# Algomorph/LevelSetFusion-Python

Measured on AMD Instinct MI355X. Metric: voxel-warp-updates/sec, higher is better.
Workload: dtype f32

## Files before the change

### include/lsf_hip.h

```cpp
#ifndef LSF_HIP_H
#define LSF_HIP_H

#include <stdint.h>

#ifdef __cplusplus
extern "C" {
#endif

#define LSF_ABI_VERSION 4
#define LSF_MAX_KERNEL_TAPS 31

#define LSF_ERR_BAD_ARGUMENT (-1)
#define LSF_ERR_BAD_DIMS (-2)
#define LSF_ERR_KERNEL_TOO_LONG (-3)
#define LSF_ERR_RCCL_UNAVAILABLE (-4)
#define LSF_ERR_RCCL_FAILED (-5)
#define LSF_ERR_NOT_RESIDENT (-6)

typedef struct lsf_grid {
    int32_t dims;
    int32_t nz, ny, nx;
    int32_t z_begin, z_end;
    int32_t z_global_offset;
    int32_t y_global_offset;
// ... 110 lines not shown
    double isomorphic_enforcement_factor_f64;
    float rate;
    float data_term_weight;
    float smoothing_term_weight;
    float level_set_term_weight;
    float isomorphic_enforcement_factor;
    float killing_c1;
    int32_t smoothing_method;
    int32_t data_method;
    int32_t level_set_enabled;
    int32_t energy_mode;
    int32_t zero_gradient_on_snap;
    int32_t reserved;
} lsf_slavcheva_params;

int lsf_slavcheva_gradient(const float *live, const float *canonical, const float *warp_prev_planar,
                           float *g_out_planar, const lsf_grid *grid, const lsf_slavcheva_params *params,
                           const lsf_gate *gate, lsf_iteration_record *record, const int32_t *band_list,
                           int64_t band_count, void *stream);

#define LSF_BAND_ALL 0
#define LSF_BAND_INTERIOR 1
#define LSF_BAND_BOUNDARY 2

int64_t lsf_band_scratch_elements(const lsf_grid *grid);
int lsf_band_count(const float *live, const float *canonical, const lsf_grid *grid, int32_t subset,
                   int32_t *scratch, int64_t *count_out, void *stream);
int lsf_band_list_fill(const float *live, const float *canonical, const lsf_grid *grid, int32_t subset,
                       const int32_t *scratch, int32_t *list, void *stream);

int64_t lsf_state_prepare_scratch_elements(const lsf_grid *grid);
int lsf_state_pack_needed(const float *live, float *state_a, float *state_b, const lsf_grid *grid, int32_t *scratch,
                          int32_t reach, int32_t invert, void *stream);

int lsf_band_list_fill_prepared(const lsf_grid *grid, int32_t subset, const int32_t *scratch, int32_t *list,
                                void *stream);
int lsf_state_prepare(const float *live, const float *canonical, float *state_a, float *state_b,
                      const lsf_grid *grid, int32_t *scratch, int64_t *counts_out, void *stream);
int lsf_state_pack(const float *live, const float *warp_planar, float *state_a, float *state_b,
                   const lsf_grid *grid, void *stream);
int lsf_state_unpack(const float *state, float *live_out, float *warp_planar_out, float *warp_interleaved_out,
                     const lsf_grid *grid, void *stream);
int64_t lsf_state_finalize_scratch_elements(const lsf_grid *grid);
int lsf_state_finalize(const float *state, const float *canonical, float *live_out, float *warp_planar_out,
                       float *warp_interleaved_out, const lsf_grid *grid, float lower_threshold,
                       double *statistics16, double *scratch, void *stream);
int lsf_planar_finalize(const float *live, const float *warp_planar, const float *canonical, float *live_out,
                        float *warp_interleaved_out, const lsf_grid *grid, float lower_threshold,
                        double *statistics16, double *scratch, void *stream);

int lsf_state_finalize_listed(const float *state, const float *canonical, float *live_out, float *warp_interleaved_out,
                              const lsf_grid *grid, const int32_t *const *band_lists, const int64_t *band_counts,
                              int32_t n_lists, int64_t opposite_count, int64_t first_opposite, float lower_threshold,
                              double *statistics16, double *scratch, const int32_t *skip_flag,
                              const lsf_iteration_record *guard_records, int32_t guard_count, float guard_limit,
                              void *stream);
int lsf_slavcheva_state_iteration(const float *state_in, const float *canonical, float *state_out,
                                  const lsf_grid *grid, const lsf_slavcheva_params *params, const lsf_gate *gate,
                                  lsf_iteration_record *record, const int32_t *band_list, int64_t band_count,
                                  int32_t band_subset, void *stream);

typedef struct lsf_band_box {
    int32_t origin;
    int32_t reserved;
    uint64_t mask;
} lsf_band_box;
// ... 292 lines not shown
```

### levelsetfusion-python_amd/_lib.py

```python
import ctypes
import os

import torch

from ._build import LIB_PATH

c_float_p = ctypes.c_void_p

MAX_KERNEL_TAPS = 31
ABI_VERSION = 4
HEADER_ABI_HASH = "bc02ed0838831b36"

ERRORS = {-1: "LSF_ERR_BAD_ARGUMENT", -2: "LSF_ERR_BAD_DIMS", -3: "LSF_ERR_KERNEL_TOO_LONG",
          -4: "LSF_ERR_RCCL_UNAVAILABLE", -5: "LSF_ERR_RCCL_FAILED", -6: "LSF_ERR_NOT_RESIDENT"}

SMOOTHING_TIKHONOV, SMOOTHING_KILLING = 0, 1
DATA_BASIC, DATA_THRESHOLDED_FDM = 0, 2
ENERGY_NONE, ENERGY_DIRECT, ENERGY_VECTORIZED = 0, 1, 2
GATE_HIERARCHICAL, GATE_SLAVCHEVA, GATE_OPEN = 0, 1, 2


class Grid(ctypes.Structure):
    _fields_ = [("dims", ctypes.c_int32), ("nz", ctypes.c_int32), ("ny", ctypes.c_int32), ("nx", ctypes.c_int32),
                ("z_begin", ctypes.c_int32), ("z_end", ctypes.c_int32), ("z_global_offset", ctypes.c_int32),
                ("y_global_offset", ctypes.c_int32), ("energy_z_begin", ctypes.c_int32), ("energy_z_end", ctypes.c_int32),
                ("ny_global", ctypes.c_int32), ("energy_y_begin", ctypes.c_int32), ("energy_y_end", ctypes.c_int32)]


BAND_ALL, BAND_INTERIOR, BAND_BOUNDARY = 0, 1, 2
RECORD_SLOTS = 8


class RecordSlot(ctypes.Structure):
    _fields_ = [("max_packed", ctypes.c_uint64), ("data_energy", ctypes.c_double),
                ("smoothing_energy", ctypes.c_double), ("level_set_energy", ctypes.c_double),
                ("pad", ctypes.c_uint64 * 508)]


class IterationRecord(ctypes.Structure):
    _fields_ = [("slot", RecordSlot * RECORD_SLOTS)]


RECORD_BYTES = ctypes.sizeof(IterationRecord)
SLOT_WORDS = ctypes.sizeof(RecordSlot) // 8
# ... 146 lines not shown
    "lsf_target_arch": (ctypes.c_char_p, []),
    "lsf_build_id": (ctypes.c_char_p, []),
    "lsf_abi_hash": (ctypes.c_char_p, []),
    "lsf_deinterleave": (ctypes.c_int, [_vp, _vp, _i64, _i32, _vp]),
    "lsf_interleave": (ctypes.c_int, [_vp, _vp, _i64, _i32, _vp]),
    "lsf_halo_copy": (ctypes.c_int, [_vp, _vp, _vp, _vp, _P(Grid), _i32, _i32, _i32, _i32, _i32, _vp]),
    "lsf_warp_field": (ctypes.c_int, [_vp, _vp, _vp, _P(Grid), _f32, _vp]),
    "lsf_warp_field_advanced": (ctypes.c_int, [_vp, _vp, _vp, _vp, _vp, _P(Grid), _i32, _vp]),
    "lsf_pack_live_gradient": (ctypes.c_int, [_vp, _vp, _P(Grid), _vp]),
    "lsf_restrict_mean": (ctypes.c_int, [_vp, _vp, _P(Grid), _i32, _vp]),
    "lsf_prolong_repeat": (ctypes.c_int, [_vp, _vp, _P(Grid), _vp]),
    "lsf_upsample2x_linear": (ctypes.c_int, [_vp, _vp, _P(Grid), _i32, _vp]),
    "lsf_downsample2x_linear": (ctypes.c_int, [_vp, _vp, _P(Grid), _i32, _vp]),
    "lsf_convolve_axis": (ctypes.c_int, [_vp, _vp, _vp, _P(Grid), _i32, _i32, _P(ctypes.c_double), _i32,
                                         _P(Gate), _vp]),
    "lsf_convolve_xy": (ctypes.c_int, [_vp, _vp, _P(Grid), _i32, _P(ctypes.c_double), _i32, _P(Gate), _vp]),
    "lsf_convolve_axis_update": (ctypes.c_int, [_vp, _vp, _vp, ctypes.c_float, _P(Grid), _i32, _i32, _P(ctypes.c_double),
                                                _i32, _P(Gate), _vp]),
    "lsf_convolve_xyz": (ctypes.c_int, [_vp, _vp, _vp, _f32, _P(Grid), _i32, _P(ctypes.c_double), _i32, _P(Gate),
                                        _vp]),
    "lsf_hier_iteration": (ctypes.c_int, [_vp, _vp, _vp, _vp, _vp, _P(Grid), _P(HierParams), _P(Gate), _vp, _vp]),
    "lsf_hier_update": (ctypes.c_int, [_vp, _vp, _P(Grid), _f32, _P(Gate), _vp, _vp]),
    "lsf_hier_level_run_2d": (ctypes.c_int, [_vp, _vp, _vp, _vp, _vp, _vp, _P(Grid), _P(HierParams), _P(ctypes.c_double),
                                            _i32, _vp, _i32, _i32, ctypes.c_float, _vp]),
    "lsf_slavcheva_gradient": (ctypes.c_int, [_vp, _vp, _vp, _vp, _P(Grid), _P(SlavchevaParams), _P(Gate), _vp,
                                              _vp, _i64, _vp]),
    "lsf_convolve_axis_listed": (ctypes.c_int, [_vp, _vp, _vp, _P(Grid), _i32, _i32, _P(ctypes.c_double), _i32,
                                                _P(Gate), _vp, _i64, _vp]),
    "lsf_state_prepare_scratch_elements": (ctypes.c_int64, [_P(Grid)]),
    "lsf_band_list_fill_prepared": (ctypes.c_int, [_P(Grid), _i32, _vp, _vp, _vp]),
    "lsf_state_prepare": (ctypes.c_int, [_vp, _vp, _vp, _vp, _P(Grid), _vp, _vp, _vp]),
    "lsf_state_pack": (ctypes.c_int, [_vp, _vp, _vp, _vp, _P(Grid), _vp]),
    "lsf_state_pack_needed": (ctypes.c_int, [_vp, _vp, _vp, _P(Grid), _vp, _i32, _i32, _vp]),
    "lsf_state_unpack": (ctypes.c_int, [_vp, _vp, _vp, _vp, _P(Grid), _vp]),
    "lsf_state_finalize_scratch_elements": (ctypes.c_int64, [_P(Grid)]),
    "lsf_state_finalize": (ctypes.c_int, [_vp, _vp, _vp, _vp, _vp, _P(Grid), _f32, _vp, _vp, _vp]),
    "lsf_planar_finalize": (ctypes.c_int, [_vp, _vp, _vp, _vp, _vp, _P(Grid), _f32, _vp, _vp, _vp]),
    "lsf_state_finalize_listed": (ctypes.c_int, [_vp, _vp, _vp, _vp, _P(Grid), _P(ctypes.c_void_p), _P(_i64), _i32,
                                                 _i64, _i64, _f32, _vp, _vp, _vp, _vp, _i32, _f32, _vp]),
    "lsf_slavcheva_state_iteration": (ctypes.c_int, [_vp, _vp, _vp, _P(Grid), _P(SlavchevaParams), _P(Gate), _vp,
                                                     _vp, _i64, _i32, _vp]),
    "lsf_band_boxes_scratch_elements": (ctypes.c_int64, [_P(Grid)]),
    "lsf_band_boxes_count": (ctypes.c_int, [_P(Grid), ctypes.c_int32, _vp, _vp, _vp, _vp]),
    "lsf_band_boxes_fill": (ctypes.c_int, [_P(Grid), ctypes.c_int32, _vp, _vp, _vp, _vp]),
    "lsf_band_boxes_canonical": (ctypes.c_int, [_vp, _P(Grid), _vp, ctypes.c_int64, _vp, _vp]),
    "lsf_slavcheva_state_iteration_boxes": (ctypes.c_int, [_vp, _vp, _vp, _P(Grid), _P(SlavchevaParams), _P(Gate), _vp, _vp,
                                                           _i64, _vp]),
    "lsf_state_run_begin": (ctypes.c_int, [_P(StateRun), _vp]),
    "lsf_state_run_finish": (ctypes.c_int, [_P(StateRun), _P(SlavchevaParams), _vp, _vp, _vp, _vp, _vp, _i32, _P(RunLoop), _vp,
                                            _f32, _vp, _vp, _vp, _vp, _P(StateRunResult), _vp]),
    "lsf_sobolev_run_finish": (ctypes.c_int, [_P(StateRun), _P(SlavchevaParams), _P(ctypes.c_double), _i32, _vp, _vp, _vp, _vp,
                                              _vp, _vp, _vp, _i32, _P(RunLoop), _vp, _f32, _vp, _vp, _vp, _vp,
                                              _P(StateRunResult), _vp]),
    "lsf_slab_run_begin": (ctypes.c_int, [_P(SlabRun), _vp]),
    "lsf_slab_run_finish": (ctypes.c_int, [_P(SlabRun), _vp, _P(SlavchevaParams), _vp, _vp, _vp, _vp, _vp, _i32, _vp, _vp, _vp,
                                           _P(StateRunResult), _vp]),
    "lsf_band_scratch_elements": (ctypes.c_int64, [_P(Grid)]),
    "lsf_band_count": (ctypes.c_int, [_vp, _vp, _P(Grid), _i32, _vp, _vp, _vp]),
    "lsf_band_list_fill": (ctypes.c_int, [_vp, _vp, _P(Grid), _i32, _vp, _vp, _vp]),
    "lsf_records_decode": (ctypes.c_int, [_vp, _i32, _i32, _i32, _vp, _vp, _vp, _vp]),
    "lsf_merge_sorted_runs": (ctypes.c_int, [_P(_vp), _P(_i64), _P(_vp), _P(_i64), _P(_vp), _i32, _vp]),
    "lsf_slab_unique_id": (ctypes.c_int, [ctypes.c_char_p, _vp]),
    "lsf_slab_comm_create": (ctypes.c_int, [ctypes.c_char_p, _vp, _i32, _i32, _P(_vp)]),
    "lsf_slab_comm_destroy": (ctypes.c_int, [_vp]),
    "lsf_slab_comm_info": (ctypes.c_int, [_vp, _P(_i32), _P(_i32)]),
    "lsf_slab_face_counts_begin": (ctypes.c_int, [_vp, _P(_i64)]),
# ... 76 lines not shown
```

### levelsetfusion-python_amd/csrc/lsf_device.h

```cpp
#pragma once

#include <hip/hip_runtime.h>
#include <cstdlib>
#include <stdint.h>

#include "../../include/lsf_hip.h"

namespace lsf {

constexpr int kWave = 64;
constexpr int kBlock = 256;
constexpr int kCuBlock = 1024;
constexpr int kMaxBlockWaves = kCuBlock / kWave;

struct FastDiv {
    unsigned d, m, l;
};

__host__ inline FastDiv make_fast_div(unsigned d) {
    FastDiv f;
    f.d = d;
    f.l = 0;
    while ((1ull << f.l) < d) ++f.l;
    f.m = (unsigned)(((1ull << 32) * ((1ull << f.l) - d)) / d + 1ull);
// ... 502 lines not shown
    return (float)__builtin_fma(-2.0, (double)a0, (double)ap + (double)am);
}

__device__ inline bool gate_closed(const lsf_gate& gate) {
    if (!gate.prev_record || gate.mode == LSF_GATE_OPEN) return false;
    unsigned long long p = 0ull;
#pragma unroll
    for (int k = 0; k < LSF_RECORD_SLOTS; ++k) {
        const unsigned long long q = gate.prev_record->slot[k].max_packed;
        p = q > p ? q : p;
    }
    if (p == 0ull) return true;
    float m = unpack_max_value(p);
    if (gate.mode == LSF_GATE_HIERARCHICAL) return m < gate.a;
    return !(gate.a < m && m < gate.b);
}

__device__ inline lsf_record_slot* record_slot(lsf_iteration_record* r) {
    return &r->slot[blockIdx.x % LSF_RECORD_SLOTS];
}

__device__ inline unsigned long long* record_max(lsf_iteration_record* r) {
    return reinterpret_cast<unsigned long long*>(&record_slot(r)->max_packed);
}

__host__ inline lsf_gate gate_or_open(const lsf_gate* gate) {
    return gate ? *gate : lsf_gate{nullptr, 0, 0.0f, 0.0f};
}

inline hipStream_t as_stream(void* s) { return reinterpret_cast<hipStream_t>(s); }

inline int launch_status() { return (int)hipGetLastError(); }

}
```

### levelsetfusion-python_amd/csrc/lsf_slavcheva.hip

```cpp
#include "lsf_device.h"

using namespace lsf;

#include "lsf_slavcheva_terms.h"

using namespace lsf::slav;

namespace {


template <int D, int SMOOTH, bool LEVELSET, int DATA, int ENERGY>
__device__ inline void voxel_gradient(const float* __restrict__ live, const float* __restrict__ canonical,
                                      const float* __restrict__ warp_prev, const Grid& g, const Params& p, int x,
                                      int y, int z, int i, float (&gv)[3], double (&en)[3]) {
    gv[0] = gv[1] = gv[2] = 0.0f;
    const float l = live[i], cn = canonical[i];
    if (fabsf(l) == 1.0f && fabsf(cn) == 1.0f) return;
    const bool interior = x > 0 && x < g.nx - 1 && y > 0 && y < g.ny - 1 && (D == 2 || (z > 0 && z < g.nz - 1));
    if (g.fast_ok && __all(interior)) {
        const NbhFast<D> n(live, warp_prev, g, x, y, z);
        band_voxel_gradient<D, SMOOTH, LEVELSET, DATA, ENERGY>(n, p, l, cn, gv, en);
    } else {
        const Nbh<D> n(live, warp_prev, g, x, y, z);
        band_voxel_gradient<D, SMOOTH, LEVELSET, DATA, ENERGY>(n, p, l, cn, gv, en);
// ... 350 lines not shown
    if (a < 2u) {
        const int* __restrict__ sums = sums_base + (size_t)a * stride;
#pragma unroll
        for (unsigned k = 0; k < 4u; ++k) sum += i + k < n ? sums[i + k] : 0;
    } else {
#pragma unroll
        for (unsigned k = 0; k < 4u; ++k)
            if (i + k < n) {
                sum += opposite[2 * (i + k)];
                first = min(first, opposite[2 * (i + k) + 1]);
            }
    }
    for (int d = kWave / 2; d > 0; d >>= 1) {
        sum += __shfl_down(sum, d, kWave);
        first = min(first, __shfl_down(first, d, kWave));
    }
    if ((t & (kWave - 1)) == 0) {
        s_sum[t / kWave] = sum;
        s_first[t / kWave] = first;
    }
    __syncthreads();
    if (t == 0) {
        for (int k = 1; k < 1024 / kWave; ++k) {
            sum += s_sum[k];
            first = min(first, s_first[k]);
        }
        tile_out[(size_t)a * tiles + tile] = sum;
        if (a == 2u) tile_out[(size_t)3 * tiles + tile] = first;
    }
}

__global__ __launch_bounds__(1024) void band_scan_tiles_kernel(int* __restrict__ sums_base, unsigned n, unsigned stride,
                                                               const int* __restrict__ tile_out, unsigned tiles,
                                                               long long* __restrict__ totals) {
    const unsigned tile = blockIdx.x, a = blockIdx.y, t = threadIdx.x, lane = t & (kWave - 1), wave = t / kWave;
    if (a == 2u) {
        if (tile == 0u && t == 0u) {
            long long sum = 0;
            int first = 0x7fffffff;
            for (unsigned k = 0; k < tiles; ++k) {
                sum += tile_out[(size_t)2 * tiles + k];
                first = min(first, tile_out[(size_t)3 * tiles + k]);
            }
            totals[2] = sum;
            totals[3] = first == 0x7fffffff ? -1 : first;
        }
        return;
    }
    __shared__ int wave_total[1024 / kWave];
    int* __restrict__ sums = sums_base + (size_t)a * stride;
    int carry = 0;
    for (unsigned k = 0; k < tile; ++k) carry += tile_out[(size_t)a * tiles + k];
    const unsigned i = tile * kScanTile + 4u * t;
    int v[4];
#pragma unroll
    for (int k = 0; k < 4; ++k) v[k] = i + k < n ? sums[i + k] : 0;
    const int mine = v[0] + v[1] + v[2] + v[3];
    int inclusive = mine;
#pragma unroll
    for (int d = 1; d < kWave; d <<= 1) {
        const int up = __shfl_up(inclusive, d, kWave);
        if ((int)lane >= d) inclusive += up;
    }
    if (lane == kWave - 1) wave_total[wave] = inclusive;
    __syncthreads();
    int before = 0, whole = 0;
#pragma unroll
    for (int w = 0; w < 1024 / kWave; ++w) {
        const int x = wave_total[w];
        before += w < (int)wave ? x : 0;
// ... 181 lines not shown
    }
    const bool any = __any(hit);
    if (lane == 0) needed[c] = any ? 1 : 0;
}

constexpr int kPackChunks = 1;
__global__ __launch_bounds__(kBlock) void state_pack_needed_kernel(const float* __restrict__ live, vf4* __restrict__ a,
                                                                   vf4* __restrict__ b, unsigned n, unsigned chunks,
                                                                   const int* __restrict__ needed, int want) {
    const int t = threadIdx.x;
    int verdict[kPackChunks];
#pragma unroll
    for (int k = 0; k < kPackChunks; ++k) {
        const unsigned c = blockIdx.x * kPackChunks + k;
        verdict[k] = c < chunks ? needed[c] : -1;
    }
#pragma unroll
    for (int k = 0; k < kPackChunks; ++k) {
        if (verdict[k] != want) continue;
        const unsigned c = blockIdx.x * kPackChunks + k;
#pragma unroll
        for (int j = 0; j < 4; ++j) {
            const unsigned v = c * kBandChunk + j * kBlock + t;
            if (v < n) {
                vf4 o;
                o.x = live[v]; o.y = 0.0f; o.z = 0.0f; o.w = 0.0f;
                if (a) a[v] = o;
                if (b) b[v] = o;
            }
        }
    }
}



__global__ __launch_bounds__(kBlock) void band_fill_from_masks_kernel(const unsigned long long* __restrict__ masks,
                                                                      const int* __restrict__ block_sums, int which,
                                                                      int* __restrict__ list, unsigned chunks) {
    const int lane = threadIdx.x % kWave;
    const unsigned chunk = blockIdx.x * (kBlock / kWave) + threadIdx.x / kWave;
    if (chunk >= chunks) return;
    const unsigned long long mine = lane < 16 ? masks[((size_t)chunk * 16 + lane) * 2 + which] : 0ull;
    if (__ballot(mine != 0ull) == 0ull) return;
    int at = block_sums[chunk];
#pragma unroll
    for (int w = 0; w < 16; ++w) {
        const unsigned lo = (unsigned)__shfl((int)(unsigned)mine, w, kWave);
        const unsigned hi = (unsigned)__shfl((int)(unsigned)(mine >> 32), w, kWave);
        const unsigned long long m = ((unsigned long long)hi << 32) | lo;
        if ((m >> lane) & 1ull)
            list[at + __popcll(m & ((1ull << lane) - 1ull))] = (int)(chunk * kBandChunk + w * kWave + lane);
        at += __popcll(m);
    }
}

}

static inline bool band_subset_ok(int32_t subset) {
    return subset == LSF_BAND_ALL || subset == LSF_BAND_INTERIOR || subset == LSF_BAND_BOUNDARY;
}

extern "C" int lsf_slavcheva_gradient(const float* live, const float* canonical, const float* warp_prev_planar,
                                      float* g_out_planar, const lsf_grid* grid, const lsf_slavcheva_params* params,
                                      const lsf_gate* gate, lsf_iteration_record* record, const int32_t* band_list,
                                      int64_t band_count, void* stream) {
    if (int e = check_grid(grid)) return e;
    if (!live || !canonical || !warp_prev_planar || !params || !record || !g_out_planar ||
// ... 216 lines not shown
extern "C" int lsf_band_boxes_count(const lsf_grid* grid, int32_t subset, const int32_t* prepare_scratch,
                                    int32_t* box_scratch, int64_t* count_out, void* stream) {
    if (int e = check_grid(grid)) return e;
    if (!boxes_ok(grid)) return LSF_ERR_BAD_DIMS;
    if (!prepare_scratch || !box_scratch || !count_out || (subset != LSF_BAND_INTERIOR && subset != LSF_BAND_ALL))
        return LSF_ERR_BAD_ARGUMENT;
    unsigned first, n, chunks;
    band_range(grid, first, n, chunks);
    const unsigned n_boxes = n / 64, groups = (n_boxes + kBoxGroup - 1) / kBoxGroup;
    hipStream_t s = as_stream(stream);
    hipLaunchKernelGGL(band_boxes_kernel<false>, dim3(groups), dim3(kBlock), 0, s,
                       prepare_masks(const_cast<int32_t*>(prepare_scratch), chunks), n_boxes, grid->nx / 4, grid->ny / 4,
                       grid->nx, grid->ny, subset == LSF_BAND_ALL, box_scratch, (lsf_band_box*)nullptr);
    hipLaunchKernelGGL(band_scan_kernel, dim3(1), dim3(1024), 0, s, box_scratch, groups, 0u, 1u, (long long*)count_out,
                       (const int*)nullptr);
    return launch_status();
}

extern "C" int lsf_band_boxes_fill(const lsf_grid* grid, int32_t subset, const int32_t* prepare_scratch,
                                   const int32_t* box_scratch, lsf_band_box* boxes, void* stream) {
    if (int e = check_grid(grid)) return e;
    if (!boxes_ok(grid)) return LSF_ERR_BAD_DIMS;
    if (!prepare_scratch || !box_scratch || !boxes || (subset != LSF_BAND_INTERIOR && subset != LSF_BAND_ALL))
        return LSF_ERR_BAD_ARGUMENT;
    unsigned first, n, chunks;
    band_range(grid, first, n, chunks);
    const unsigned n_boxes = n / 64, groups = (n_boxes + kBoxGroup - 1) / kBoxGroup;
    hipLaunchKernelGGL(band_boxes_kernel<true>, dim3(groups), dim3(kBlock), 0, as_stream(stream),
                       prepare_masks(const_cast<int32_t*>(prepare_scratch), chunks), n_boxes, grid->nx / 4, grid->ny / 4,
                       grid->nx, grid->ny, subset == LSF_BAND_ALL, const_cast<int32_t*>(box_scratch), boxes);
    return launch_status();
}

extern "C" int lsf_state_prepare(const float* live, const float* canonical, float* state_a, float* state_b,
                                 const lsf_grid* grid, int32_t* scratch, int64_t* counts_out, void* stream) {
    if (int e = check_grid(grid, true)) return e;
    if (!live || !canonical || (!state_a && state_b) || !scratch || !counts_out) return LSF_ERR_BAD_ARGUMENT;
    if (grid->z_begin != 0 || grid->z_end != grid->nz) return LSF_ERR_BAD_ARGUMENT;
    unsigned first, n, chunks;
    band_range(grid, first, n, chunks);
    hipStream_t s = as_stream(stream);
    int* sums_interior = scratch;
    int* sums_boundary = scratch + (chunks + 1);
    const bool wide = grid->nx % 4 == 0 && ((uintptr_t)live | (uintptr_t)canonical) % 16 == 0;
    if (wide)
        hipLaunchKernelGGL(state_prepare4_kernel, dim3((chunks + kPrepareChunksPerBlock - 1) / kPrepareChunksPerBlock),
                           dim3(kBlock), 0, s, reinterpret_cast<const vf4*>(live), reinterpret_cast<const vf4*>(canonical),
                           reinterpret_cast<vf4*>(state_a), reinterpret_cast<vf4*>(state_b), n, chunks, make_grid(grid),
                           grid->dims, sums_interior, sums_boundary, prepare_masks(scratch, chunks),
                           prepare_opposite(scratch, chunks), prepare_nonempty(scratch, chunks));
    else
        hipLaunchKernelGGL(state_prepare_kernel, dim3(chunks), dim3(kBlock), 0, s, live, canonical,
                           reinterpret_cast<vf4*>(state_a), reinterpret_cast<vf4*>(state_b), n, make_grid(grid), grid->dims,
                           sums_interior, sums_boundary, prepare_masks(scratch, chunks), prepare_opposite(scratch, chunks),
                           prepare_nonempty(scratch, chunks));
    const unsigned tiles = prepare_scan_tiles(chunks) > 0u ? prepare_scan_tiles(chunks) : 1u;
    hipLaunchKernelGGL(band_tile_totals_kernel, dim3(tiles, 3), dim3(1024), 0, s, scratch, chunks, chunks + 1,
                       (const int*)prepare_opposite(scratch, chunks), prepare_tile_totals(scratch, chunks), tiles);
    hipLaunchKernelGGL(band_scan_tiles_kernel, dim3(tiles, 3), dim3(1024), 0, s, scratch, chunks, chunks + 1,
                       (const int*)prepare_tile_totals(scratch, chunks), tiles, (long long*)counts_out);
    return launch_status();
}

extern "C" int lsf_state_pack_needed(const float* live, float* state_a, float* state_b, const lsf_grid* grid,
                                     int32_t* scratch, int32_t reach, int32_t invert, void* stream) {
    if (int e = check_grid(grid, true)) return e;
    if (!live || (!state_a && !state_b) || !scratch || reach < 1 || reach > 8) return LSF_ERR_BAD_ARGUMENT;
    if (grid->z_begin != 0 || grid->z_end != grid->nz) return LSF_ERR_BAD_ARGUMENT;
    unsigned first, n, chunks;
    band_range(grid, first, n, chunks);
    if (!invert)
        hipLaunchKernelGGL(chunk_needed_kernel, dim3((chunks + kBlock / kWave - 1) / (kBlock / kWave)), dim3(kBlock), 0, as_stream(stream),
                           chunks, (long long)grid->nx, (long long)grid->nx * grid->ny, grid->dims, reach,
                           prepare_nonempty(scratch, chunks), prepare_needed(scratch, chunks));
    hipLaunchKernelGGL(state_pack_needed_kernel, dim3((chunks + kPackChunks - 1) / kPackChunks), dim3(kBlock), 0,
                       as_stream(stream), live, reinterpret_cast<vf4*>(state_a), reinterpret_cast<vf4*>(state_b), n, chunks,
                       prepare_needed(scratch, chunks), invert ? 0 : 1);
    return launch_status();
}

extern "C" int lsf_band_list_fill(const float* live, const float* canonical, const lsf_grid* grid, int32_t subset,
                                  const int32_t* scratch, int32_t* list, void* stream) {
    if (int e = check_grid(grid)) return e;
    if (!live || !canonical || !scratch || !list || !band_subset_ok(subset)) return LSF_ERR_BAD_ARGUMENT;
    unsigned first, n, chunks;
    if (!band_range(grid, first, n, chunks)) return 0;
    hipLaunchKernelGGL(band_list_kernel<true>, dim3(chunks), dim3(kBlock), 0, as_stream(stream), live, canonical, first, n,
                       make_grid(grid), grid->dims, subset, const_cast<int32_t*>(scratch), list);
    return launch_status();
}
```

### levelsetfusion-python_amd/csrc/lsf_slavcheva_run.hip

```cpp
#include "lsf_device.h"

#include <cstring>

using namespace lsf;

namespace {

__global__ __launch_bounds__(kBlock) void records_used_words_kernel(const long long* __restrict__ records,
                                                                    const long long* __restrict__ statistics16,
                                                                    long long* __restrict__ out, int n_slots, int tail) {
    const int k = blockIdx.x * kBlock + threadIdx.x;
    if (k < n_slots * 4) out[k] = records[(long long)(k >> 2) * (sizeof(lsf_record_slot) / 8) + (k & 3)];
    else if (tail && k < n_slots * 4 + 16) out[k] = statistics16 ? statistics16[k - n_slots * 4] : 0ll;
}

inline hipEvent_t thread_event() {
    thread_local hipEvent_t events[64] = {};
    int dev = 0;
    if (hipGetDevice(&dev) != hipSuccess || dev < 0 || dev >= 64) return nullptr;
    if (!events[dev] && hipEventCreateWithFlags(&events[dev], hipEventDisableTiming) != hipSuccess) events[dev] = nullptr;
    return events[dev];
}

inline bool run_ok(const lsf_state_run* r) {
    return r && r->live && r->canonical && r->state[0] && r->state[1] && r->state[0] != r->state[1] && r->prepare_scratch &&
           r->totals_device && r->totals_host && r->sparse_reach >= 0 && r->sparse_reach <= 8;
}

}

extern "C" int lsf_state_run_begin(const lsf_state_run* run, void* stream) {
    if (!run_ok(run)) return LSF_ERR_BAD_ARGUMENT;
    const lsf_grid* g = &run->grid;
    if (int e = check_grid(g)) return e;
    if (g->z_begin != 0 || g->z_end != g->nz) return LSF_ERR_BAD_ARGUMENT;
    hipStream_t s = as_stream(stream);
    const bool sparse = run->sparse_reach > 0;
    float* b_in_pass = (sparse || run->second_state_late) ? nullptr : run->state[1];
    if (int e = lsf_state_prepare(run->live, run->canonical, sparse ? nullptr : run->state[0], b_in_pass, g,
                                  run->prepare_scratch, run->totals_device, stream))
        return e;
    if (run->box_scratch) {
        if (int e = lsf_band_boxes_count(g, run->box_all ? LSF_BAND_ALL : LSF_BAND_INTERIOR, run->prepare_scratch, run->box_scratch,
                                         run->totals_device + 4, stream))
            return e;
    } else if (hipMemsetAsync(run->totals_device + 4, 0, sizeof(int64_t), s) != hipSuccess) {
        return (int)hipGetLastError();
    }
    if (hipMemcpyAsync(run->totals_host, run->totals_device, 5 * sizeof(int64_t), hipMemcpyDeviceToHost, s) != hipSuccess)
        return (int)hipGetLastError();
    hipEvent_t sizes = thread_event();
    if (!sizes) return (int)hipGetLastError();
    int status = 0;
    if (hipEventRecord(sizes, s) != hipSuccess) status = (int)hipGetLastError();
    if (!status && sparse)
        status = lsf_state_pack_needed(run->live, run->state[0], run->state[1], g, run->prepare_scratch, run->sparse_reach, 0,
                                       stream);
    else if (!status && run->second_state_late)
        status = lsf_state_pack(run->live, nullptr, run->state[1], nullptr, g, stream);
    if (!status && hipEventSynchronize(sizes) != hipSuccess) status = (int)hipGetLastError();
    return status;
}

extern "C" int lsf_state_run_finish(const lsf_state_run* run, const lsf_slavcheva_params* params, int32_t* list_interior,
                                    int32_t* list_boundary, lsf_band_box* boxes, float* box_canonical,
                                    lsf_iteration_record* records, int32_t iterations, const lsf_run_loop* loop,
                                    float* live_out, float lower_threshold, double* statistics16,
                                    double* finalize_scratch, int64_t* words_device, int64_t* words_host,
                                    lsf_state_run_result* result, void* stream) {
    if (!run_ok(run) || !params || !records || iterations < 1 || !live_out || !words_device || !words_host || !result ||
        (statistics16 && !finalize_scratch) || !result->max_value || !result->argmax ||
        !result->energies3 || !result->executed)
        return LSF_ERR_BAD_ARGUMENT;
    if (loop && (loop->min_iterations < 1 || loop->check_interval < 1 ||
                 (loop->max_iterations > loop->min_iterations ? loop->max_iterations : loop->min_iterations) != iterations))
        return LSF_ERR_BAD_ARGUMENT;
    if (run->box_all && boxes) return LSF_ERR_BAD_ARGUMENT;
    const lsf_grid* g = &run->grid;
    if (int e = check_grid(g)) return e;
    const int64_t n_interior = run->totals_host[0], n_boundary = run->totals_host[1];
    if (n_interior < 0 || n_boundary < 0 || n_interior > 0x7fffffffll || n_boundary > 0x7fffffffll ||
        (n_interior && !list_interior) || (n_boundary && !list_boundary))
        return LSF_ERR_BAD_ARGUMENT;
    hipStream_t s = as_stream(stream);
    const int32_t* lists[2];
    int64_t counts[2];
    int32_t subsets[2];
    int n_lists = 0;
    if (n_interior) {
        if (int e = lsf_band_list_fill_prepared(g, LSF_BAND_INTERIOR, run->prepare_scratch, list_interior, stream)) return e;
// ... 195 lines not shown
```

### levelsetfusion-python_amd/engine_run.py

```python
import ctypes

import numpy as np
import torch

from . import _lib, device as dev
from .engine_common import _Counted
from .engine_outcome import _RunLog, _RunOutcome


class _SparseStateExceeded(Exception):
    """a call whose ping-pong states were initialised near the band only (dev.StatePrepare(sparse_reach=...)) met a warp
    update that can read beyond that; nothing of the caller's has been modified (SlavchevaEngine.optimize repeats the
    call on fully initialised states and keeps doing so for this optimizer)"""


class _RunGradient:

    def __init__(self, g4):
        self._g4 = g4

    def final_gradient_planar(self, dims):
        return self._g4[..., :dims].movedim(-1, 0).contiguous()


class RunMixin:

    def _optimize_run(self, live, canonical, grid, finalize, sobolev=False):
        live_out, lower_threshold, statistics = finalize
        iterations = max(self.min_iterations, self.max_iterations)
        loop = None
        if self.min_iterations < iterations:
            loop = _lib.RunLoop(self.min_iterations, self.max_iterations, self.lo, self.hi, self.check_interval, 0)
        device = live.device
        n = dev.n_voxels(grid)
        whole = dev.full_range(grid)
        sparse = (self.sparse_reach > 0 and n >= self.sparse_min_voxels and not self.sparse_disabled)
        self.last_call.sparse_states = sparse
        self.last_call.library_run = True
        usable = (live_out is not None and live_out.is_cuda and live_out.dtype == torch.float32
                  and live_out.is_contiguous() and tuple(live_out.shape) == tuple(live.shape))
        target = live_out if usable else torch.empty_like(live)
        if target is not live:
            target.copy_(live)
        states = [torch.empty(tuple(live.shape) + (4,), dtype=torch.float32, device=device) for _ in range(2)]
        scratch = torch.empty(int(_lib.lib.lsf_state_prepare_scratch_elements(ctypes.byref(whole))), dtype=torch.int32,
                              device=device)
        totals = torch.empty(5, dtype=torch.int64, device=device)
        totals_host = dev.pinned_scratch("run totals", 5, torch.int64)
        run = _lib.StateRun()
        run.live, run.canonical = dev._ptr(live, n, "live"), dev._ptr(canonical, n, "canonical")
        run.state[0], run.state[1] = states[0].data_ptr(), states[1].data_ptr()
        run.prepare_scratch, run.totals_device, run.totals_host = scratch.data_ptr(), totals.data_ptr(), totals_host.data_ptr()
        run.grid = whole
        run.sparse_reach = self.sparse_reach if sparse else 0
        run.second_state_late = int(not sparse and n <= dev.StatePrepare.SPLIT_MAX_VOXELS)
        count_boxes = sobolev or (dev.boxes_ok(whole) and (self.box_walk is True or
                                                           (self.box_walk is None and n >= self.box_walk_min_voxels)))
        run.box_all = int(sobolev)
        box_scratch = None
        if count_boxes:
            box_scratch = torch.empty(int(_lib.lib.lsf_band_boxes_scratch_elements(ctypes.byref(whole))),
                                      dtype=torch.int32, device=device)
            run.box_scratch = box_scratch.data_ptr()
        stream = dev.stream_ptr()
        _lib.check(_lib.lib.lsf_state_run_begin(ctypes.byref(run), stream), "lsf_state_run_begin")
        n_interior, n_boundary, opposite, first_opposite, n_boxes = totals_host.tolist()
        lists = torch.empty(max(n_interior + n_boundary, 1), dtype=torch.int32, device=device)
        boxes = box_canonical = None
        if sobolev:
            boxes = torch.empty((max(n_boxes, 1), 2), dtype=torch.int64, device=device)
            list_all = torch.empty(max(n_interior + n_boundary, 1), dtype=torch.int32, device=device) \
                if n_interior and n_boundary else None
            g4 = self._sobolev_gradient_buffers(live, whole, lists, n_interior + n_boundary)
            taps = np.ascontiguousarray(np.asarray(self.sobolev_kernel, dtype=np.float64))
            self.last_call.sobolev_boxes = True
        elif n_boxes and (self.box_walk is True or 32 * n_interior > self.box_walk_min_band_bytes):
            boxes = torch.empty((n_boxes, 2), dtype=torch.int64, device=device)
# ... 88 lines not shown
```

### levelsetfusion-python_amd/engine_slavcheva.py

```python
import ctypes

import numpy as np
import torch

from . import _lib, device as dev, engine_options
from .engine_common import _Counted
from .engine_focus import FocusMixin
from .engine_outcome import SlavchevaOutcome
from .engine_run import RunMixin, _SparseStateExceeded
from .engine_slab import SlabMixin, _HaloTooNarrow
from .engine_sobolev import PlanarSobolevMixin, _SobolevStatePlan


class SlavchevaEngine(RunMixin, SlabMixin, PlanarSobolevMixin, FocusMixin):

    def __init__(self, direct, level_set_term_enabled, sobolev_smoothing_enabled, data_term_method,
                 smoothing_term_method, gradient_descent_rate, data_term_weight, smoothing_term_weight,
                 isomorphic_enforcement_factor, level_set_term_weight, lower_threshold, upper_threshold,
                 max_iterations, min_iterations, sobolev_kernel, compute_energies=True, check_interval=32,
                 comm=None, options=None):
        self.direct = bool(direct)
        self.sobolev = bool(sobolev_smoothing_enabled)
        self.sobolev_kernel = sobolev_kernel
        if self.sobolev and sobolev_kernel is None:
            raise ValueError("sobolev_smoothing_enabled requires a sobolev_kernel")
        lam = float(isomorphic_enforcement_factor)
        smoothing = smoothing_term_method if self.direct else _lib.SMOOTHING_TIKHONOV
        data = data_term_method if self.direct else _lib.DATA_BASIC
        level_set = bool(level_set_term_enabled) and self.direct
        energy = _lib.ENERGY_NONE if not compute_energies else \
            (_lib.ENERGY_DIRECT if self.direct else _lib.ENERGY_VECTORIZED)
        self.params = _lib.SlavchevaParams(lam, float(gradient_descent_rate), float(data_term_weight),
                                           float(smoothing_term_weight), float(level_set_term_weight), lam,
                                           float(np.float32(-2.0 * (1.0 + lam))), int(smoothing), int(data),
                                           int(level_set), int(energy), int(self.direct), 0)
        self.weights = (float(data_term_weight), float(smoothing_term_weight), float(level_set_term_weight))
        self.lo, self.hi = float(lower_threshold), float(upper_threshold)
        self.max_iterations, self.min_iterations = int(max_iterations), int(min_iterations)
        self.check_interval = max(1, int(check_interval))
        self.comm = comm
        engine_options.apply(self, engine_options.SLAVCHEVA_DEFAULTS, options)
        self.last_call = engine_options.new_call_report()
        self.sparse_disabled = False
        self.iteration_count = 0
        self.log = None
        self._gradient_state = None
        self.iteration_hook = None

    def _grid(self, live):
        if self.comm is not None and self.comm.active:
            L = self.comm.layout
            if L.axis == 1:
                if live.dim() != 3 or live.shape[1] != L.n_local:
                    raise ValueError("y-slab runs need a 3-D local field with %d rows, got %r"
                                     % (L.n_local, tuple(live.shape)))
                g = dev.make_grid(live.shape)
                g.y_global_offset, g.ny_global = L.global_offset, L.n_global
                g.energy_y_begin, g.energy_y_end = L.begin, L.end
                return g
            if live.dim() != 3 or live.shape[0] != L.nz_local:
                raise ValueError("slab runs need a 3-D local field with %d slices, got %r"
                                 % (L.nz_local, tuple(live.shape)))
            return dev.make_grid(live.shape, L.z_begin, L.z_end, L.z_global_offset)
        return dev.make_grid(live.shape)

    def _slab(self):
        return self.comm is not None and self.comm.active

    def _gate_for(self, records, i):
        return None if i < self.min_iterations else dev.make_gate(records, i - 1, _lib.GATE_SLAVCHEVA, self.lo,
                                                                  self.hi)

    def _enqueue_state_iteration(self, i, states, limit):
        f = self._fast
        s_in, s_out = f.p_state[i % 2], f.p_state[(i + 1) % 2]
        gate_ref = None if i < self.min_iterations else f.gate_ref(i - 1)
# ... 289 lines not shown
```

Baseline: 524.1 billion.

## Pack sparse state from dilated band bitmasks and fold box-total zeroing into scan

Adds a kernel that builds the set of needed voxels by dilating the band bitmasks over a reach-sized neighbourhood using 64-bit word shifts. It then writes only those voxels into the two state buffers, replacing the older pack_needed path in the sparse run setup. It also zeroes the box-total counter inside the scan kernel instead of issuing a separate memset. The dilation costs extra bit arithmetic per word, but it avoids separate scratch passes and a launch. A debug option to pre-fill the state buffers is added but is off by default.

```diff
diff --git a/include/lsf_hip.h b/include/lsf_hip.h
--- a/include/lsf_hip.h
+++ b/include/lsf_hip.h
@@ -166,6 +166,8 @@
 int64_t lsf_state_prepare_scratch_elements(const lsf_grid *grid);
 int lsf_state_pack_needed(const float *live, float *state_a, float *state_b, const lsf_grid *grid, int32_t *scratch,
                           int32_t reach, int32_t invert, void *stream);
+int lsf_state_pack_near_band(const float *live, float *state_a, float *state_b, const lsf_grid *grid, const int32_t *scratch,
+                             int32_t reach, uint64_t *needed_words, void *stream);
 
 int lsf_band_list_fill_prepared(const lsf_grid *grid, int32_t subset, const int32_t *scratch, int32_t *list,
                                 void *stream);
diff --git a/levelsetfusion-python_amd/_lib.py b/levelsetfusion-python_amd/_lib.py
--- a/levelsetfusion-python_amd/_lib.py
+++ b/levelsetfusion-python_amd/_lib.py
@@ -9,7 +9,7 @@
 
 MAX_KERNEL_TAPS = 31
 ABI_VERSION = 4
-HEADER_ABI_HASH = "bc02ed0838831b36"
+HEADER_ABI_HASH = "ef0d30eb84eeba6d"
 
 ERRORS = {-1: "LSF_ERR_BAD_ARGUMENT", -2: "LSF_ERR_BAD_DIMS", -3: "LSF_ERR_KERNEL_TOO_LONG",
           -4: "LSF_ERR_RCCL_UNAVAILABLE", -5: "LSF_ERR_RCCL_FAILED", -6: "LSF_ERR_NOT_RESIDENT"}
@@ -222,6 +222,7 @@
     "lsf_state_prepare": (ctypes.c_int, [_vp, _vp, _vp, _vp, _P(Grid), _vp, _vp, _vp]),
     "lsf_state_pack": (ctypes.c_int, [_vp, _vp, _vp, _vp, _P(Grid), _vp]),
     "lsf_state_pack_needed": (ctypes.c_int, [_vp, _vp, _vp, _P(Grid), _vp, _i32, _i32, _vp]),
+    "lsf_state_pack_near_band": (ctypes.c_int, [_vp, _vp, _vp, _P(Grid), _vp, _i32, _vp, _vp]),
     "lsf_state_unpack": (ctypes.c_int, [_vp, _vp, _vp, _vp, _P(Grid), _vp]),
     "lsf_state_finalize_scratch_elements": (ctypes.c_int64, [_P(Grid)]),
     "lsf_state_finalize": (ctypes.c_int, [_vp, _vp, _vp, _vp, _vp, _P(Grid), _f32, _vp, _vp, _vp]),
diff --git a/levelsetfusion-python_amd/csrc/lsf_device.h b/levelsetfusion-python_amd/csrc/lsf_device.h
--- a/levelsetfusion-python_amd/csrc/lsf_device.h
+++ b/levelsetfusion-python_amd/csrc/lsf_device.h
@@ -558,4 +558,7 @@
 
 inline int launch_status() { return (int)hipGetLastError(); }
 
-}
+int state_prepare_launch(const float* live, const float* canonical, float* state_a, float* state_b, const lsf_grid* grid,
+                         int32_t* scratch, int64_t* counts_out, bool zero_box_total, void* stream);
+
+}
diff --git a/levelsetfusion-python_amd/csrc/lsf_slavcheva.hip b/levelsetfusion-python_amd/csrc/lsf_slavcheva.hip
--- a/levelsetfusion-python_amd/csrc/lsf_slavcheva.hip
+++ b/levelsetfusion-python_amd/csrc/lsf_slavcheva.hip
@@ -406,10 +406,11 @@
 
 __global__ __launch_bounds__(1024) void band_scan_tiles_kernel(int* __restrict__ sums_base, unsigned n, unsigned stride,
                                                                const int* __restrict__ tile_out, unsigned tiles,
-                                                               long long* __restrict__ totals) {
+                                                               long long* __restrict__ totals, int zero_box_total) {
     const unsigned tile = blockIdx.x, a = blockIdx.y, t = threadIdx.x, lane = t & (kWave - 1), wave = t / kWave;
     if (a == 2u) {
         if (tile == 0u && t == 0u) {
+            if (zero_box_total) totals[4] = 0;
             long long sum = 0;
             int first = 0x7fffffff;
             for (unsigned k = 0; k < tiles; ++k) {
@@ -657,7 +658,81 @@
     }
 }
 
-
+__device__ inline unsigned long long band_word(const unsigned long long* __restrict__ masks, long long q, long long words) {
+    return q >= 0 && q < words ? (masks[2 * q] | masks[2 * q + 1]) : 0ull;
+}
+
+__device__ inline unsigned long long bits_at(unsigned long long w0, unsigned long long w1, unsigned long long w2, int o) {
+    if (o >= 64) {
+        w0 = w1;
+        w1 = w2;
+        o -= 64;
+    }
+    return o == 0 ? w0 : (w0 >> o) | (w1 << (64 - o));
+}
+
+__device__ inline unsigned long long dilated_row(const unsigned long long* __restrict__ masks, long long words, long long w_bit,
+                                                 int k, int span, int reach, int dims, long long row, long long slice) {
+    const int dy = k % span - reach, dz = dims == 3 ? k / span - reach : 0;
+    const long long s = w_bit + dz * slice + dy * row - reach;
+    const long long q = s >= 0 ? s / 64 : -((-s + 63) / 64);
+    const int sh = (int)(s - q * 64);
+    const unsigned long long w0 = band_word(masks, q, words), w1 = band_word(masks, q + 1, words),
+                             w2 = band_word(masks, q + 2, words);
+    unsigned long long m = 0ull;
+    if (w0 | w1 | w2)
+        for (int dx = 0; dx < span; ++dx) m |= bits_at(w0, w1, w2, sh + dx);
+    return m;
+}
+
+__global__ __launch_bounds__(kBlock) void state_pack_near_band_kernel(const unsigned long long* __restrict__ masks,
+                                                                      const float* __restrict__ live, vf4* __restrict__ a,
+                                                                      vf4* __restrict__ b, unsigned n, unsigned chunks,
+                                                                      long long row, long long slice, int dims, int reach,
+                                                                      unsigned long long* __restrict__ needed_out) {
+    __shared__ unsigned long long s_part[kBlock / kWave][16], s_need[16], s_band[16];
+    const int t = threadIdx.x, word = t & 15, group = t >> 4, lane = t & (kWave - 1);
+    const unsigned chunk = blockIdx.x;
+    const long long words = (long long)chunks * 16, w_index = (long long)chunk * 16 + word;
+    const int span = 2 * reach + 1, rows = dims == 3 ? span * span : span;
+    unsigned long long m = 0ull;
+    for (int k = group; k < rows; k += 32) {
+        const unsigned long long m0 = dilated_row(masks, words, w_index * 64, k, span, reach, dims, row, slice);
+        const unsigned long long m1 =
+            k + 16 < rows ? dilated_row(masks, words, w_index * 64, k + 16, span, reach, dims, row, slice) : 0ull;
+        m |= m0 | m1;
+    }
+#pragma unroll
+    for (int d = 16; d < kWave; d <<= 1) {
+        const unsigned lo = (unsigned)__shfl_xor((int)(unsigned)m, d, kWave);
+        const unsigned hi = (unsigned)__shfl_xor((int)(unsigned)(m >> 32), d, kWave);
+        m |= ((unsigned long long)hi << 32) | lo;
+    }
+    if (lane < 16) s_part[t / kWave][word] = m;
+    __syncthreads();
+    if (t < 16) {
+        m = s_part[0][word] | s_part[1][word] | s_part[2][word] | s_part[3][word];
+        const long long first_bit = w_index * 64;
+        if (first_bit + 64 > (long long)n) m &= first_bit < (long long)n ? (1ull << ((long long)n - first_bit)) - 1ull : 0ull;
+        s_need[word] = m;
+        s_band[word] = band_word(masks, w_index, words);
+        if (needed_out) needed_out[w_index] = m;
+    }
+    __syncthreads();
+    if (!(a || b)) return;
+#pragma unroll
+    for (int j = 0; j < 4; ++j) {
+        const unsigned local = j * kBlock + t, v = chunk * kBandChunk + local;
+        const unsigned long long bit = 1ull << (local & 63u);
+        const unsigned long long need = s_need[local >> 6];
+        if (v < n && (need & bit)) {
+            vf4 o;
+            o.x = live[v]; o.y = 0.0f; o.z = 0.0f; o.w = 0.0f;
+            if (a) a[v] = o;
+            if (b && !(s_band[local >> 6] & bit)) b[v] = o;
+        }
+    }
+}
 
 __global__ __launch_bounds__(kBlock) void band_fill_from_masks_kernel(const unsigned long long* __restrict__ masks,
                                                                       const int* __restrict__ block_sums, int which,
@@ -940,8 +1015,8 @@
     return launch_status();
 }
 
-extern "C" int lsf_state_prepare(const float* live, const float* canonical, float* state_a, float* state_b,
-                                 const lsf_grid* grid, int32_t* scratch, int64_t* counts_out, void* stream) {
+int lsf::state_prepare_launch(const float* live, const float* canonical, float* state_a, float* state_b, const lsf_grid* grid,
+                              int32_t* scratch, int64_t* counts_out, bool zero_box_total, void* stream) {
     if (int e = check_grid(grid, true)) return e;
     if (!live || !canonical || (!state_a && state_b) || !scratch || !counts_out) return LSF_ERR_BAD_ARGUMENT;
     if (grid->z_begin != 0 || grid->z_end != grid->nz) return LSF_ERR_BAD_ARGUMENT;
@@ -966,7 +1041,27 @@
     hipLaunchKernelGGL(band_tile_totals_kernel, dim3(tiles, 3), dim3(1024), 0, s, scratch, chunks, chunks + 1,
                        (const int*)prepare_opposite(scratch, chunks), prepare_tile_totals(scratch, chunks), tiles);
     hipLaunchKernelGGL(band_scan_tiles_kernel, dim3(tiles, 3), dim3(1024), 0, s, scratch, chunks, chunks + 1,
-                       (const int*)prepare_tile_totals(scratch, chunks), tiles, (long long*)counts_out);
+                       (const int*)prepare_tile_totals(scratch, chunks), tiles, (long long*)counts_out, zero_box_total ? 1 : 0);
+    return launch_status();
+}
+
+extern "C" int lsf_state_prepare(const float* live, const float* canonical, float* state_a, float* state_b,
+                                 const lsf_grid* grid, int32_t* scratch, int64_t* counts_out, void* stream) {
+    return lsf::state_prepare_launch(live, canonical, state_a, state_b, grid, scratch, counts_out, false, stream);
+}
+
+extern "C" int lsf_state_pack_near_band(const float* live, float* state_a, float* state_b, const lsf_grid* grid,
+                                        const int32_t* scratch, int32_t reach, uint64_t* needed_words, void* stream) {
+    if (int e = check_grid(grid)) return e;
+    if (!scratch || reach < 1 || reach > 8 || ((state_a || state_b) && !live) || (state_a && state_a == state_b))
+        return LSF_ERR_BAD_ARGUMENT;
+    if (grid->z_begin != 0 || grid->z_end != grid->nz) return LSF_ERR_BAD_ARGUMENT;
+    unsigned first, n, chunks;
+    if (!band_range(grid, first, n, chunks)) return 0;
+    hipLaunchKernelGGL(state_pack_near_band_kernel, dim3(chunks), dim3(kBlock), 0, as_stream(stream),
+                       prepare_masks(const_cast<int32_t*>(scratch), chunks), live, reinterpret_cast<vf4*>(state_a),
+                       reinterpret_cast<vf4*>(state_b), n, chunks, (long long)grid->nx, (long long)grid->nx * grid->ny,
+                       grid->dims, reach, reinterpret_cast<unsigned long long*>(needed_words));
     return launch_status();
 }
 
diff --git a/levelsetfusion-python_amd/csrc/lsf_slavcheva_run.hip b/levelsetfusion-python_amd/csrc/lsf_slavcheva_run.hip
--- a/levelsetfusion-python_amd/csrc/lsf_slavcheva_run.hip
+++ b/levelsetfusion-python_amd/csrc/lsf_slavcheva_run.hip
@@ -37,16 +37,13 @@
     hipStream_t s = as_stream(stream);
     const bool sparse = run->sparse_reach > 0;
     float* b_in_pass = (sparse || run->second_state_late) ? nullptr : run->state[1];
-    if (int e = lsf_state_prepare(run->live, run->canonical, sparse ? nullptr : run->state[0], b_in_pass, g,
-                                  run->prepare_scratch, run->totals_device, stream))
-        return e;
-    if (run->box_scratch) {
+    if (int e = state_prepare_launch(run->live, run->canonical, sparse ? nullptr : run->state[0], b_in_pass, g,
+                                     run->prepare_scratch, run->totals_device, !run->box_scratch, stream))
+        return e;
+    if (run->box_scratch)
         if (int e = lsf_band_boxes_count(g, run->box_all ? LSF_BAND_ALL : LSF_BAND_INTERIOR, run->prepare_scratch, run->box_scratch,
                                          run->totals_device + 4, stream))
             return e;
-    } else if (hipMemsetAsync(run->totals_device + 4, 0, sizeof(int64_t), s) != hipSuccess) {
-        return (int)hipGetLastError();
-    }
     if (hipMemcpyAsync(run->totals_host, run->totals_device, 5 * sizeof(int64_t), hipMemcpyDeviceToHost, s) != hipSuccess)
         return (int)hipGetLastError();
     hipEvent_t sizes = thread_event();
@@ -54,8 +51,8 @@
     int status = 0;
     if (hipEventRecord(sizes, s) != hipSuccess) status = (int)hipGetLastError();
     if (!status && sparse)
-        status = lsf_state_pack_needed(run->live, run->state[0], run->state[1], g, run->prepare_scratch, run->sparse_reach, 0,
-                                       stream);
+        status = lsf_state_pack_near_band(run->live, run->state[0], run->state[1], g, run->prepare_scratch, run->sparse_reach,
+                                          nullptr, stream);
     else if (!status && run->second_state_late)
         status = lsf_state_pack(run->live, nullptr, run->state[1], nullptr, g, stream);
     if (!status && hipEventSynchronize(sizes) != hipSuccess) status = (int)hipGetLastError();
diff --git a/levelsetfusion-python_amd/engine_run.py b/levelsetfusion-python_amd/engine_run.py
--- a/levelsetfusion-python_amd/engine_run.py
+++ b/levelsetfusion-python_amd/engine_run.py
@@ -43,6 +43,9 @@
         if target is not live:
             target.copy_(live)
         states = [torch.empty(tuple(live.shape) + (4,), dtype=torch.float32, device=device) for _ in range(2)]
+        if self.state_fill_before_run is not None:
+            for state in states:
+                state.fill_(self.state_fill_before_run)
         scratch = torch.empty(int(_lib.lib.lsf_state_prepare_scratch_elements(ctypes.byref(whole))), dtype=torch.int32,
                               device=device)
         totals = torch.empty(5, dtype=torch.int64, device=device)
diff --git a/levelsetfusion-python_amd/engine_slavcheva.py b/levelsetfusion-python_amd/engine_slavcheva.py
--- a/levelsetfusion-python_amd/engine_slavcheva.py
+++ b/levelsetfusion-python_amd/engine_slavcheva.py
@@ -42,6 +42,7 @@
         engine_options.apply(self, engine_options.SLAVCHEVA_DEFAULTS, options)
         self.last_call = engine_options.new_call_report()
         self.sparse_disabled = False
+        self.state_fill_before_run = None
         self.iteration_count = 0
         self.log = None
         self._gradient_state = None
```

After: 530.3 billion (median of 6 runs). No clear change (+1.2%).
